# ginkgo-project/ginkgo

Measured on AMD Instinct MI355X. Metric: CSR SpMV GB/s (27-pt 3D Laplacian 256^3, fp64/int32), higher is better.
Workload: dtype f64

## Files before the change

ginkgo_amd/csrc/csr_offsets.hpp:

```cpp
#pragma once
#include "common.hpp"
#include <type_traits>

namespace gkoc {

constexpr int OFFS_MAX = 32;
constexpr int OFFS_TAB = OFFS_MAX + 1;

#ifdef __HIPCC__

template <typename I>
__global__ __launch_bounds__(256) void csr_offsets_build_kernel(int64_t n_rows, const I* __restrict__ row_ptrs,
                                                                const I* __restrict__ cols,
                                                                int32_t* __restrict__ seg_tab,
                                                                uint32_t* __restrict__ row_mask)
{
    const int64_t seg = int64_t(blockIdx.x) * 4 + threadIdx.x / 64;
    const int lane = threadIdx.x % 64;
    if (seg * 64 >= n_rows) return;
    const int64_t row = seg * 64 + lane;
    const bool valid = row < n_rows;
    int64_t pos = valid ? int64_t(row_ptrs[row]) : 0;
    const int64_t end = valid ? int64_t(row_ptrs[row + 1]) : 0;
    constexpr long long NONE = 0x7fffffffffffffffll;
    uint32_t mask = 0;
    int D = 0;
    int32_t my_off = 0;
    bool ok = true;
    long long last = 0;
    for (;;) {
        const long long cur = pos < end ? (long long)(cols[pos]) - (long long)(row) : NONE;
        long long m = cur;
#pragma unroll
        for (int o = 32; o > 0; o >>= 1) {
            const long long t = __shfl_xor(m, o, 64);
            m = t < m ? t : m;
        }
        if (m == NONE) break;
        if (D == OFFS_MAX || (D > 0 && m <= last) || m < -2147483648ll || m > 2147483647ll) {
            ok = false;
            break;
        }
        if (lane == D) my_off = int32_t(m);
        if (cur == m) {
            mask |= 1u << D;
            ++pos;
        }
        last = m;
        ++D;
    }
    if (!ok) D = 0;
    if (lane == 0) seg_tab[seg * OFFS_TAB] = D;
    if (lane < OFFS_MAX) seg_tab[seg * OFFS_TAB + 1 + lane] = lane < D ? my_off : 0;
    if (valid) row_mask[row] = ok ? mask : 0u;
}

__global__ __launch_bounds__(1024) void csr_offsets_finish_kernel(int64_t n_seg, const int32_t* __restrict__ seg_tab,
                                                                  const uint32_t* __restrict__ long_bits,
                                                                  uint32_t* __restrict__ skip,
                                                                  unsigned long long* __restrict__ count)
{
    __shared__ long long part[16];
    const int64_t n_words = (n_seg + 31) / 32;
    long long mine = 0;
    for (int64_t w = threadIdx.x; w < n_words; w += 1024) {
        uint32_t bits = 0;
        for (int j = 0; j < 32; ++j) {
            const int64_t s = w * 32 + j;
            if (s < n_seg && seg_tab[s * OFFS_TAB] > 0) bits |= 1u << j;
        }
        mine += __popc(bits);
        skip[w] = long_bits != nullptr ? (bits | long_bits[w]) : bits;
    }
    const long long total = block_sum<1024>(mine, part);
    if (threadIdx.x == 0) *count = static_cast<unsigned long long>(total);
}

template <typename T, bool ADV, bool DOT>
__global__ __launch_bounds__(64, 2) void csr_spmv_pipe3_kernel_offsets(
    int32_t n_rows, int32_t n_cols, int64_t n_segments, int spw, const int32_t* __restrict__ row_ptrs,
    const T* __restrict__ vals, const T* __restrict__ x, T* __restrict__ c, const T* __restrict__ alpha_p,
    const T* __restrict__ beta_p, const int32_t* __restrict__ seg_tab, const uint32_t* __restrict__ row_mask,
    T* __restrict__ dot_partial)
{
    constexpr int GR = 64;
    constexpr int E = 16 / sizeof(T);
    constexpr int CAP = GR * OFFS_MAX;
    constexpr int NL = CAP / (64 * E) + 1;
    constexpr int GPS = 64 / GR;
    typedef T VT __attribute__((ext_vector_type(E)));
    __shared__ __attribute__((aligned(16))) T stage[CAP + E];

    const int lane = threadIdx.x;
    const int64_t wave_id = blockIdx.x;
    const int64_t sb = wave_id * spw;
    const int n_units = int((sb + spw < n_segments ? int64_t(spw) : n_segments - sb)) * GPS;
    T alpha = T(1), beta = T(0);
    if (ADV) {
        alpha = alpha_p[0];
        beta = beta_p[0];
    }
    T dot_acc = T(0);

    struct unit {
        int D;
        int row0;
        int k0a, len;
        const int32_t* tab;
    };
    auto unit_of = [&](int u) {
        unit q;
        const int64_t s = sb + u / GPS;
        q.row0 = int(s * 64) + (u % GPS) * GR;
        q.tab = seg_tab + s * OFFS_TAB;
        q.D = (u < n_units && q.row0 < n_rows) ? q.tab[0] : 0;
        q.k0a = q.len = 0;
        if (q.D > 0) {
            const int last = q.row0 + GR < n_rows ? q.row0 + GR : n_rows;
            const int k0 = row_ptrs[q.row0];
            const int k1 = row_ptrs[last];
            q.k0a = k0 & ~(E - 1);
            q.len = k1 > k0 ? k1 - q.k0a : 0;
            if (q.len > CAP + E - 1) q.len = CAP + E - 1;
        }
        return q;
    };
    VT v[NL];
    auto load_vals = [&](const unit& q) {
        const int last_chunk = (q.len - 1) & ~(E - 1);
#pragma unroll
        for (int t = 0; t < NL; ++t) {
            const int k = (t * 64 + lane) * E;
            v[t] = *reinterpret_cast<const VT*>(vals + (int64_t(q.k0a) + (k < last_chunk ? k : last_chunk)));
        }
    };
    auto group = [&](auto nd_c, const unit& cur, const unit& nxt, int u) {
        constexpr int ND = decltype(nd_c)::value;
        const int row = cur.row0 + lane;
        const bool valid = lane < GR && row < n_rows;
        const int last = cur.row0 + GR < n_rows ? cur.row0 + GR : n_rows;
        const int rs = row_ptrs[valid ? row : last] - cur.k0a;
        uint32_t mask = row_mask[valid ? row : cur.row0];
        if (!valid) mask = 0u;
        T sum = T(0), bdot = T(0);
        if (ADV && beta != T(0)) sum = c[valid ? row : cur.row0] * beta;
        if (DOT) bdot = x[valid ? row : cur.row0];
        const int ncm1 = n_cols - 1;
        T xv[ND];
#pragma unroll
        for (int d = 0; d < ND; ++d) {
            const int idx = int(uint32_t(row) + uint32_t(cur.tab[1 + d]));
            xv[d] = x[idx < 0 ? 0 : (idx > ncm1 ? ncm1 : idx)];
        }
        if (cur.len > 0) {
#pragma unroll
            for (int t = 0; t < NL; ++t) {
                const int k = (t * 64 + lane) * E;
                if (k < cur.len) *reinterpret_cast<VT*>(&stage[k]) = v[t];
            }
        }
        wave_lds_sync();
        if (nxt.D > 0 && nxt.len > 0) load_vals(nxt);
#pragma unroll
        for (int d0 = 0; d0 < ND; d0 += 8) {
            T val[8];
#pragma unroll
            for (int i = 0; i < 8; ++i) {
                const int pos = rs + __popc(mask & ((1u << (d0 + i)) - 1u));
                val[i] = stage[pos];
            }
#pragma unroll
            for (int i = 0; i < 8; ++i) {
                asm volatile("" : "+v"(val[i]));
            }
#pragma unroll
            for (int i = 0; i < 8; ++i) {
                const T pr = ADV ? (alpha * val[i]) * xv[d0 + i] : val[i] * xv[d0 + i];
                sum = ((mask >> (d0 + i)) & 1u) != 0 ? sum + pr : sum;
            }
        }
        if (valid) c[row] = sum;
        if constexpr (DOT) {
            const T term = bdot * sum;
            if (valid) dot_acc += term;
        }
        wave_lds_sync();
    };

    unit cur = unit_of(0);
    if (cur.D > 0 && cur.len > 0) load_vals(cur);
    for (int u = 0; u < n_units; ++u) {
        const unit nxt = unit_of(u + 1);
        if (cur.D > 8) {
            group(std::integral_constant<int, OFFS_MAX>{}, cur, nxt, u);
        } else if (cur.D > 0) {
            group(std::integral_constant<int, 8>{}, cur, nxt, u);
        } else if (nxt.D > 0 && nxt.len > 0) {
            load_vals(nxt);
        }
        cur = nxt;
    }
    if constexpr (DOT) {
        dot_acc = wave_sum(dot_acc);
        if (lane == 0) dot_partial[wave_id] = dot_acc;
    }
}

#endif

}
```

ginkgo_amd/csrc/csr_spmv.hip:

```cpp
#include <algorithm>
#include <atomic>
#include <map>
#include <mutex>
#include <tuple>
#include <type_traits>
#include <vector>

#include "common.hpp"
#include "csr_long_rows.hpp"
#include "csr_offsets.hpp"
#include "csr_spmv_multi.hpp"
#include "csr_spmv_pipe.hpp"
#include "fused.hpp"

namespace gkoc {
namespace {

std::mutex g_long_mtx;
struct long_entry {
    csr_long_info info;
    std::vector<std::pair<hipStream_t, void*>> partials;
};
std::map<std::tuple<int, const void*, int64_t>, long_entry> g_long_cache;
std::atomic<int> g_long_cached{0};
constexpr size_t long_cache_cap = 128;
constexpr int64_t long_list_cap = 4096;

thread_local bool t_long_releasing = false;

void long_info_release(long_entry& en)
{
    csr_long_info& f = en.info;
    t_long_releasing = true;
    if (f.bits) (void)gkoc_free(f.bits);
    if (f.list) (void)gkoc_free(f.list);
    for (auto& sp : en.partials) (void)gkoc_free(sp.second);
    en.partials.clear();
    f = csr_long_info{};
    t_long_releasing = false;
}

bool stream_is_capturing(hipStream_t st)
{
    hipStreamCaptureStatus cap = hipStreamCaptureStatusNone;
    if (hipStreamIsCapturing(st, &cap) != hipSuccess || cap != hipStreamCaptureStatusNone) {
        (void)hipGetLastError();
        return true;
    }
    return false;
}

void long_partial_for(long_entry& en, hipStream_t st, csr_long_info* out)
{
    *out = en.info;
    if (en.info.count <= 0) return;
    for (auto& sp : en.partials) {
        if (sp.first == st) {
            out->partial = sp.second;
            return;
        }
    }
    void* p = nullptr;
    if (stream_is_capturing(st) ||
        gkoc_malloc(&p, size_t(en.info.count) * LONG_MAX_PER_SEG * LONG_PARTS * 8) != GKOC_OK) {
        (void)hipGetLastError();
        *out = csr_long_info{};
        out->nnz = en.info.nnz;
        return;
    }
    en.partials.emplace_back(st, p);
    out->partial = p;
}

template <typename T, typename I>
int long_info_of(gkoc_stream_t s, int64_t n_rows, const I* row_ptrs, csr_long_info* out)
{
    int dev = 0;
    GKOC_HIP(hipGetDevice(&dev));
    const auto key = std::make_tuple(dev, static_cast<const void*>(row_ptrs), n_rows);
    std::lock_guard<std::mutex> g(g_long_mtx);
    auto it = g_long_cache.find(key);
    if (it != g_long_cache.end()) {
        long_partial_for(it->second, as_stream(s), out);
        return GKOC_OK;
    }
    if (stream_is_capturing(as_stream(s))) {
        *out = csr_long_info{};
        return GKOC_OK;
    }
    if (g_long_cache.size() >= long_cache_cap) {
        auto oldest = g_long_cache.begin();
        for (auto jt = g_long_cache.begin(); jt != g_long_cache.end(); ++jt) {
            if (jt->second.info.seq < oldest->second.info.seq) oldest = jt;
        }
        if (oldest->second.info.count > 0) GKOC_HIP(hipDeviceSynchronize());
        long_info_release(oldest->second);
        g_long_cache.erase(oldest);
    }
    csr_long_info f;
    static uint64_t arrivals = 0;
    f.seq = ++arrivals;
    const int64_t n_seg = ceildiv(n_rows, int64_t(64));
    const size_t bit_bytes = size_t(ceildiv(n_seg, int64_t(32))) * 4;
    const size_t list_bytes = size_t(1 + long_list_cap) * 8;
    void *bits = nullptr, *list = nullptr;
    GKOC_TRY(gkoc_malloc(&bits, bit_bytes));
    if (gkoc_malloc(&list, list_bytes) != GKOC_OK) {
        t_long_releasing = true;
        (void)gkoc_free(bits);
        t_long_releasing = false;
        return GKOC_E_INVALID;
    }
    hipStream_t st = as_stream(s);
    unsigned long long count = 0;
    I nnz_dev = I(0);
    bool ok = hipMemsetAsync(bits, 0, bit_bytes, st) == hipSuccess && hipMemsetAsync(list, 0, 8, st) == hipSuccess;
    if (ok) {
        csr_long_row_scan_kernel<I><<<dim3(unsigned(ceildiv(n_seg, int64_t(4)))), dim3(256), 0, st>>>(
            n_rows, row_ptrs, static_cast<uint32_t*>(bits), static_cast<unsigned long long*>(list), long_list_cap);
        ok = hipGetLastError() == hipSuccess &&
             hipMemcpyAsync(&count, list, 8, hipMemcpyDeviceToHost, st) == hipSuccess &&
             hipMemcpyAsync(&nnz_dev, row_ptrs + n_rows, sizeof(I), hipMemcpyDeviceToHost, st) == hipSuccess &&
             hipStreamSynchronize(st) == hipSuccess;
    }
    if (ok) f.nnz = int64_t(nnz_dev);
    if (!ok || count == 0 || int64_t(count) > long_list_cap) {
        (void)hipGetLastError();
        t_long_releasing = true;
        (void)gkoc_free(bits);
        (void)gkoc_free(list);
        t_long_releasing = false;
    } else {
        f.count = int64_t(count);
        f.bits = static_cast<uint32_t*>(bits);
        f.list = static_cast<unsigned long long*>(list);
    }
    long_entry& en = g_long_cache[key];
    en.info = f;
    g_long_cached.store(int(g_long_cache.size()));
    long_partial_for(en, st, out);
    return GKOC_OK;
}

}

void csr_long_rows_forget(const void* ptr)
{
    if (ptr == nullptr || t_long_releasing || g_long_cached.load(std::memory_order_relaxed) == 0) return;
    std::vector<long_entry> gone;
    {
        std::lock_guard<std::mutex> g(g_long_mtx);
        for (auto it = g_long_cache.begin(); it != g_long_cache.end();) {
            if (std::get<1>(it->first) == ptr) {
                gone.push_back(it->second);
                it = g_long_cache.erase(it);
            } else {
                ++it;
            }
        }
        g_long_cached.store(int(g_long_cache.size()));
    }
    for (auto& en : gone) {
        if (en.info.count > 0) (void)hipDeviceSynchronize();
        long_info_release(en);
    }
}

std::atomic<int> g_csr_offsets_cached{0};

namespace {

template <int N>
using int_c = std::integral_constant<int, N>;

struct segment_plan {
    int64_t n_seg;
    int spw;
    int64_t n_waves;
};

int plan_segments(int64_t n_rows, segment_plan* plan, int64_t forced_spw = 0)
{
    const int64_t n_seg = ceildiv(n_rows, 64);
    const int spw = (forced_spw == 1 || forced_spw == 2) ? int(forced_spw) : (n_seg < 65536 ? 1 : 2);
    const int64_t n_waves = ceildiv(n_seg, spw);
    GKOC_REQUIRE(n_waves < (int64_t(1) << 31), GKOC_E_NOT_SUPPORTED, "more than 2^31 row segments");
    *plan = segment_plan{n_seg, spw, n_waves};
    return GKOC_OK;
}

template <typename F>
void with_store_mode(int spw, F&& launch)
{
    if (spw == 2) {
        launch(int_c<0x2000>{});
    } else {
        launch(int_c<0x1000>{});
    }
}

template <typename V, typename I>
bool streams_aligned(const V* vals, const I* cols, int E)
{
    return reinterpret_cast<uintptr_t>(vals) % (E * sizeof(V)) == 0 &&
           reinterpret_cast<uintptr_t>(cols) % (E * sizeof(I)) == 0;
}

template <typename T>
struct pipe_layout {
    static constexpr int EV = 32 / sizeof(T);
    static constexpr int RINGV = 8192 / sizeof(T);
    static constexpr int PE = sizeof(T) == 8 ? 2 : 4, PU = sizeof(T) == 8 ? 3 : 2;
};

template <typename T, typename I, bool ADV>
int launch_csr_columns(gkoc_stream_t s, int64_t n_rows, int64_t n_cols, const T* alpha, const I* row_ptrs,
                       const I* col_idxs, const T* vals, const T* b, int64_t ldb, const T* beta, T* c,
                       int64_t ldc, int64_t nrhs)
{
    const bool idx32 = n_cols * ldb < (int64_t(1) << 32);
    const bool pairs_ok = reinterpret_cast<uintptr_t>(b) % (2 * sizeof(T)) == 0 && ldb % 2 == 0 &&
                          reinterpret_cast<uintptr_t>(c) % (2 * sizeof(T)) == 0 && ldc % 2 == 0;
    const int64_t chunk_rows = tune_value(GKOC_TUNE_MULTI_XCD_CHUNK_ROWS);
    auto launch = [&](auto nr, auto cpl, auto ku, auto pipelined) -> int {
        constexpr int NR = decltype(nr)::value, CPL = decltype(cpl)::value, KU = decltype(ku)::value;
        constexpr bool PIPE = decltype(pipelined)::value;
        constexpr int rows = 64 * CPL / NR, segs = PIPE ? 4 : 1;
        const int64_t nwg = ceildiv(ceildiv(n_rows, rows), segs);
        GKOC_REQUIRE(nwg < (int64_t(1) << 31), GKOC_E_NOT_SUPPORTED, "more than 2^31 waves");
        const dim3 grid(static_cast<unsigned>(nwg)), block(64);
        auto go = [&](auto idx) {
            constexpr bool IDX32 = decltype(idx)::value;
            if constexpr (PIPE) {
                csr_spmv_frag_pipe_kernel<T, I, ADV, NR, CPL, KU, IDX32><<<grid, block, 0, as_stream(s)>>>(
                    n_rows, row_ptrs, col_idxs, vals, b, ldb, c, ldc, static_cast<int>(nrhs), alpha, beta, segs,
                    chunk_rows / (rows * segs));
            } else {
                csr_spmv_frag_kernel<T, I, ADV, NR, CPL, KU, IDX32><<<grid, block, 0, as_stream(s)>>>(
                    n_rows, row_ptrs, col_idxs, vals, b, ldb, c, ldc, static_cast<int>(nrhs), alpha, beta,
                    chunk_rows / rows);
            }
        };
        if (idx32) {
            go(std::true_type{});
        } else {
            go(std::false_type{});
        }
        GKOC_LAUNCH_OK();
        return GKOC_OK;
    };
    if (nrhs <= 4) return launch(int_c<4>{}, int_c<1>{}, int_c<4>{}, std::true_type{});
    if (pairs_ok) return launch(int_c<8>{}, int_c<2>{}, int_c<3>{}, std::true_type{});
    return launch(int_c<8>{}, int_c<1>{}, int_c<4>{}, std::false_type{});
}

template <typename T, typename I, bool ADV>
int launch_csr_pair(gkoc_stream_t s, int64_t n_rows, const T* alpha, const I* row_ptrs, const I* col_idxs,
                    const T* vals, const T* b, int64_t ldb, const T* beta, T* c, int64_t ldc)
{
    using lay = pipe_layout<T>;
    segment_plan p;
    GKOC_TRY(plan_segments(n_rows, &p));
    const dim3 grid(static_cast<unsigned>(p.n_waves)), block(64);
    const int b_vec_ok = reinterpret_cast<uintptr_t>(b) % (2 * sizeof(T)) == 0 && ldb % 2 == 0;
    const int64_t xcd_chunk = tune_value(GKOC_TUNE_MULTI_XCD_CHUNK_ROWS) / (64 * p.spw);
    auto launch = [&](auto e, auto u) {
        csr_spmv_multi_kernel<T, I, ADV, decltype(e)::value, decltype(u)::value, lay::RINGV / 2, 2>
            <<<grid, block, 0, as_stream(s)>>>(n_rows, p.n_seg, p.spw, row_ptrs, col_idxs, vals, b, ldb, c, ldc, 2,
                                               alpha, beta, b_vec_ok, xcd_chunk);
    };
    if (tune_value(GKOC_TUNE_CSR_LOAD_GROUPS) == 1) {
        launch(int_c<lay::EV>{}, int_c<1>{});
    } else {
        launch(int_c<lay::EV / 2>{}, int_c<2>{});
    }
    GKOC_LAUNCH_OK();
    return GKOC_OK;
}

std::mutex g_off_mtx;
struct offsets_plan {
    int state = 0;
    int64_t n_seg = 0, eligible = 0;
    int32_t* seg_tab = nullptr;
    uint32_t* row_mask = nullptr;
    uint32_t* skip = nullptr;
    bool with_long = false;
    int64_t bytes = 0, products = 0;
    uint64_t seq = 0;
    size_t rp_bytes = 0, ci_bytes = 0;
};
using offsets_key = std::tuple<int, const void*, const void*, int64_t>;
std::map<offsets_key, offsets_plan> g_off_cache;
constexpr size_t offsets_cache_cap = 128;
constexpr int64_t offsets_min_share = 50;

std::vector<void*> g_off_graveyard;

void offsets_release(std::vector<offsets_plan>& gone)
{
    std::vector<void*> bufs;
    for (auto& pl : gone) {
        for (void* b : {static_cast<void*>(pl.seg_tab), static_cast<void*>(pl.row_mask), static_cast<void*>(pl.skip)}) {
            if (b) bufs.push_back(b);
        }
    }
    if (bufs.empty()) return;
    std::lock_guard<std::mutex> g(g_off_mtx);
    g_off_graveyard.insert(g_off_graveyard.end(), bufs.begin(), bufs.end());
    if (hipDeviceSynchronize() != hipSuccess) {
        (void)hipGetLastError();
        return;
    }
    for (void* b : g_off_graveyard) (void)arena_free(b);
    g_off_graveyard.clear();
}

int offsets_build(hipStream_t st, int64_t n_rows, const int32_t* row_ptrs, const int32_t* col_idxs,
                  const csr_long_info& lng, offsets_plan& pl)
{
    const int64_t n_seg = ceildiv(n_rows, int64_t(64));
    const size_t tab_bytes = size_t(n_seg) * OFFS_TAB * 4, mask_bytes = size_t(n_rows) * 4;
    const size_t skip_bytes = size_t(ceildiv(n_seg, int64_t(32))) * 4;
    void *tab = nullptr, *mask = nullptr, *skip = nullptr, *count_dev = nullptr;
    bool ok = arena_malloc(&tab, tab_bytes, GKOC_MEM_INDICES) == GKOC_OK &&
              arena_malloc(&mask, mask_bytes, GKOC_MEM_INDICES) == GKOC_OK &&
              arena_malloc(&skip, skip_bytes, GKOC_MEM_INDICES) == GKOC_OK &&
              arena_malloc(&count_dev, 8, GKOC_MEM_VECTOR) == GKOC_OK;
    unsigned long long count = 0;
    if (ok) {
        csr_offsets_build_kernel<int32_t><<<dim3(unsigned(ceildiv(n_seg, int64_t(4)))), dim3(256), 0, st>>>(
            n_rows, row_ptrs, col_idxs, static_cast<int32_t*>(tab), static_cast<uint32_t*>(mask));
        csr_offsets_finish_kernel<<<dim3(1), dim3(1024), 0, st>>>(
            n_seg, static_cast<const int32_t*>(tab), lng.count > 0 ? lng.bits : nullptr,
            static_cast<uint32_t*>(skip), static_cast<unsigned long long*>(count_dev));
        ok = hipGetLastError() == hipSuccess &&
             hipMemcpyAsync(&count, count_dev, 8, hipMemcpyDeviceToHost, st) == hipSuccess &&
             hipStreamSynchronize(st) == hipSuccess;
    }
    (void)hipGetLastError();
    if (count_dev) (void)arena_free(count_dev);
    pl.n_seg = n_seg;
    pl.eligible = ok ? int64_t(count) : 0;
    if (!ok || pl.eligible == 0 || pl.eligible * 100 < n_seg * offsets_min_share) {
        if (tab) (void)arena_free(tab);
        if (mask) (void)arena_free(mask);
        if (skip) (void)arena_free(skip);
        if (ok) pl.state = 2;
        return GKOC_OK;
    }
    pl.state = 1;
    pl.seg_tab = static_cast<int32_t*>(tab);
    pl.row_mask = static_cast<uint32_t*>(mask);
    pl.bytes = int64_t(tab_bytes + mask_bytes);
    if (pl.eligible == n_seg) {
        (void)arena_free(skip);
    } else {
        pl.skip = static_cast<uint32_t*>(skip);
        pl.with_long = lng.count > 0;
        pl.bytes += int64_t(skip_bytes);
    }
    return GKOC_OK;
}

struct evicted_plans {
    std::vector<offsets_plan> v;
    ~evicted_plans() { offsets_release(v); }
};

offsets_plan* offsets_plan_for(hipStream_t st, int64_t n_rows, int64_t n_cols, const int32_t* row_ptrs,
                               const int32_t* col_idxs, const csr_long_info& lng, std::vector<offsets_plan>* evicted)
{
    const int64_t mode = tune_value(GKOC_TUNE_CSR_OFFSETS);
    if (mode == 2 || row_ptrs == nullptr || col_idxs == nullptr || n_cols < 1 ||
        n_rows >= (int64_t(1) << 31) - 64 || n_cols >= (int64_t(1) << 31)) {
        return nullptr;
    }
    int dev = 0;
    if (hipGetDevice(&dev) != hipSuccess) return nullptr;
    const offsets_key key{dev, row_ptrs, col_idxs, n_rows};
    auto it = g_off_cache.find(key);
    if (it == g_off_cache.end()) {
        const size_t rp_bytes = arena_allocation_bytes(row_ptrs), ci_bytes = arena_allocation_bytes(col_idxs);
        if (rp_bytes == 0 || ci_bytes == 0) return nullptr;
        if (g_off_cache.size() >= offsets_cache_cap) {
            auto oldest = g_off_cache.begin();
            for (auto jt = g_off_cache.begin(); jt != g_off_cache.end(); ++jt) {
                if (jt->second.seq < oldest->second.seq) oldest = jt;
            }
            evicted->push_back(oldest->second);
            g_off_cache.erase(oldest);
        }
        static uint64_t arrivals = 0;
        offsets_plan fresh;
        fresh.seq = ++arrivals;
        fresh.rp_bytes = rp_bytes;
        fresh.ci_bytes = ci_bytes;
        it = g_off_cache.emplace(key, fresh).first;
        g_csr_offsets_cached.store(int(g_off_cache.size()));
        if (mode != 1) return nullptr;
    }
    offsets_plan& pl = it->second;
    if (pl.state == 0) {
        if (stream_is_capturing(st)) return nullptr;
        (void)offsets_build(st, n_rows, row_ptrs, col_idxs, lng, pl);
    }
    if (pl.state != 1) return nullptr;
    if (pl.skip != nullptr && pl.with_long != (lng.count > 0)) return nullptr;
    return &pl;
}

template <typename T, bool ADV, bool DOT>
void launch_offsets_kernel(hipStream_t st, const offsets_plan& pl, const segment_plan& p, int64_t n_rows,
                           int64_t n_cols, const T* alpha, const int32_t* row_ptrs, const T* vals, const T* b,
                           const T* beta, T* c, T* dot_partial)
{
    const dim3 grid(static_cast<unsigned>(p.n_waves)), block(64);
    csr_spmv_pipe3_kernel_offsets<T, ADV, DOT><<<grid, block, 0, st>>>(
        int32_t(n_rows), int32_t(n_cols), p.n_seg, p.spw, row_ptrs, vals, b, c, alpha, beta, pl.seg_tab,
        pl.row_mask, dot_partial);
}

template <typename T, typename I, bool ADV>
int launch_hub_rows(hipStream_t st, const csr_long_info& lng, int64_t n_rows, const T* alpha, const I* row_ptrs,
                    const I* col_idxs, const T* vals, const T* b, int64_t ldb, const T* beta, T* c, int64_t ldc)
{
    csr_flagged_segments_kernel<T, I, ADV><<<dim3(unsigned(lng.count * LONG_PARTS)), dim3(LONG_WG), 0, st>>>(
        n_rows, row_ptrs, col_idxs, vals, b, ldb, c, ldc, alpha, beta, lng.list, static_cast<T*>(lng.partial));
    GKOC_LAUNCH_OK();
    csr_long_rows_fold_kernel<T, I, ADV><<<dim3(unsigned(lng.count)), dim3(64), 0, st>>>(
        n_rows, row_ptrs, c, ldc, beta, lng.list, static_cast<const T*>(lng.partial));
    GKOC_LAUNCH_OK();
    return GKOC_OK;
}

template <typename T, typename I, bool ADV>
int launch_csr_single(gkoc_stream_t s, int64_t n_rows, int64_t n_cols, const T* alpha, const I* row_ptrs, const I* col_idxs,
                      const T* vals, const T* b, int64_t ldb, const T* beta, T* c, int64_t ldc, int64_t nrhs)
{
    using lay = pipe_layout<T>;
    csr_long_info lng;
    if (nrhs == 1 && tune_value(GKOC_TUNE_CSR_LONG_ROWS) != 0) {
        GKOC_TRY((long_info_of<T, I>(s, n_rows, row_ptrs, &lng)));
    }
    const uint32_t* seg_skip = lng.count > 0 ? lng.bits : nullptr;
    constexpr bool offsets_type = std::is_same<I, int32_t>::value && (sizeof(T) == 8 || sizeof(T) == 4);
    evicted_plans evicted;
    std::unique_lock<std::mutex> plan_lock(g_off_mtx, std::defer_lock);
    offsets_plan* plan = nullptr;
    if constexpr (offsets_type) {
        if (nrhs == 1 && ldb == 1 && ldc == 1 && vals != nullptr && b != nullptr &&
            reinterpret_cast<uintptr_t>(vals) % 16 == 0 && tune_value(GKOC_TUNE_CSR_OFFSETS) != 2) {
            plan_lock.lock();
            plan = offsets_plan_for(as_stream(s), n_rows, n_cols, row_ptrs, col_idxs, lng, &evicted.v);
            if (plan == nullptr) plan_lock.unlock();
        }
    }
    segment_plan p;
    GKOC_TRY(plan_segments(n_rows, &p, tune_value(GKOC_TUNE_CSR_SEGS_PER_WAVE)));
    const dim3 grid(static_cast<unsigned>(p.n_waves)), block(64);
    if constexpr (offsets_type) {
        if (plan != nullptr) {
            launch_offsets_kernel<T, ADV, false>(as_stream(s), *plan, p, n_rows, n_cols, alpha, row_ptrs, vals, b,
                                                 beta, c, static_cast<T*>(nullptr));
            GKOC_LAUNCH_OK();
            ++plan->products;
            if (plan->skip == nullptr) return GKOC_OK;
            seg_skip = plan->skip;
        }
    }
    const int64_t xcd_choice = tune_value(GKOC_TUNE_CSR_XCD_MAP);
    const int xcd_map =
        ((xcd_choice == 1 || (xcd_choice == 0 && lng.count > 0)) && p.n_waves >= 8 * 1024) ? 1 : 0;
    const bool vec_ok = streams_aligned(vals, col_idxs, lay::EV);
    const int64_t groups = tune_value(GKOC_TUNE_CSR_LOAD_GROUPS);
    const bool long_float_rows = sizeof(T) == 4 && lng.nnz > 0 && lng.nnz >= 40 * n_rows;
    with_store_mode(p.spw, [&](auto mode) {
        auto launch = [&](auto e, auto u) {
            csr_spmv_pipe3_kernel<T, I, ADV, 64, decltype(e)::value, decltype(u)::value, lay::RINGV, 1,
                                  decltype(mode)::value><<<grid, block, 0, as_stream(s)>>>(
                n_rows, p.n_seg, p.spw, row_ptrs, col_idxs, vals, b, ldb, c, ldc, static_cast<int>(nrhs), alpha,
                beta, nullptr, xcd_map, static_cast<const I*>(nullptr), static_cast<int*>(nullptr), int64_t(0),
                int64_t(0), static_cast<const uint32_t*>(nullptr), uint32_t(0), static_cast<const I*>(nullptr),
                static_cast<const I*>(nullptr), static_cast<const T*>(nullptr), static_cast<uint32_t*>(nullptr),
                uint32_t(0), 0, int64_t(-1), seg_skip);
        };
        if (!vec_ok) {
            launch(int_c<1>{}, int_c<4>{});
        } else if (groups == 3 || (groups == 0 && long_float_rows)) {
            launch(int_c<1>{}, int_c<8>{});
        } else if (groups == 4) {
            launch(int_c<2>{}, int_c<4>{});
        } else if (groups == 1 || p.n_seg < 32768) {
            launch(int_c<lay::EV>{}, int_c<1>{});
        } else {
            launch(int_c<lay::PE>{}, int_c<lay::PU>{});
        }
    });
    GKOC_LAUNCH_OK();
    if (lng.count > 0) {
        GKOC_TRY((launch_hub_rows<T, I, ADV>(as_stream(s), lng, n_rows, alpha, row_ptrs, col_idxs, vals, b, ldb,
                                             beta, c, ldc)));
    }
    return GKOC_OK;
}

template <typename T, typename I, bool ADV>
int launch_csr(gkoc_stream_t s, int64_t n_rows, int64_t n_cols, const T* alpha,
               const I* row_ptrs, const I* col_idxs, const T* vals, const T* b,
               int64_t ldb, const T* beta, T* c, int64_t ldc, int64_t nrhs)
{
    GKOC_REQUIRE(n_rows >= 0 && n_cols >= 0 && nrhs >= 0, GKOC_E_INVALID,
                 "negative dimension");
    if (n_rows == 0 || nrhs == 0) return GKOC_OK;
    GKOC_REQUIRE(row_ptrs && c, GKOC_E_INVALID, "null pointer");
    GKOC_REQUIRE(ldc >= nrhs && (n_cols == 0 || ldb >= nrhs), GKOC_E_INVALID,
                 "stride smaller than nrhs");
    if (ADV) GKOC_REQUIRE(alpha && beta, GKOC_E_INVALID, "null alpha/beta");
    if (nrhs >= 3) {
        return launch_csr_columns<T, I, ADV>(s, n_rows, n_cols, alpha, row_ptrs, col_idxs, vals, b, ldb, beta, c,
                                             ldc, nrhs);
    }
    if (nrhs == 2 && streams_aligned(vals, col_idxs, pipe_layout<T>::EV)) {
        return launch_csr_pair<T, I, ADV>(s, n_rows, alpha, row_ptrs, col_idxs, vals, b, ldb, beta, c, ldc);
    }
    return launch_csr_single<T, I, ADV>(s, n_rows, n_cols, alpha, row_ptrs, col_idxs, vals, b, ldb, beta, c, ldc, nrhs);
}

__global__ void gate_open_kernel(uint32_t* gate, uint32_t epoch)
{
    __hip_atomic_store(gate, epoch, __ATOMIC_RELEASE, __HIP_MEMORY_SCOPE_SYSTEM);
}

int64_t gated_wave_cap() { return int64_t(current_device_props().num_cu) * 8; }

bool gated_fits(int64_t n_rows, int64_t head_rows, int64_t tail_rows)
{
    if (n_rows <= 0 || head_rows < 0 || tail_rows < 0 || head_rows + tail_rows > n_rows ||
        head_rows + tail_rows == 0) {
        return false;
    }
    return ceildiv(head_rows + tail_rows, 64) <= gated_wave_cap();
}

template <typename T, typename I>
int launch_csr_gated(gkoc_stream_t s, int64_t n_rows, const I* row_ptrs, const I* col_idxs, const T* vals,
                     const I* bnd_ptrs, const I* bnd_cols, const T* bnd_vals, const T* b, T* c,
                     int64_t head_rows, int64_t tail_rows, const uint32_t* gate, uint32_t epoch,
                     uint32_t* fork_word, uint32_t fork_number, T* dot_out = nullptr, void* work = nullptr,
                     size_t work_bytes = 0)
{
    GKOC_REQUIRE(n_rows > 0 && head_rows >= 0 && tail_rows >= 0 && head_rows + tail_rows <= n_rows,
                 GKOC_E_INVALID, "bad dimensions");
    GKOC_REQUIRE(head_rows + tail_rows > 0, GKOC_E_INVALID, "no boundary rows: use gkoc_csr_spmv_*");
    GKOC_REQUIRE(row_ptrs && col_idxs && vals && bnd_ptrs && bnd_cols && bnd_vals && b && c && gate,
                 GKOC_E_INVALID, "null pointer");
    GKOC_REQUIRE(gated_fits(n_rows, head_rows, tail_rows), GKOC_E_NOT_SUPPORTED,
                 "more boundary rows than may wait on the device at once (gkoc_csr_spmv_gated_fits): "
                 "use the join-based product");
    using lay = pipe_layout<T>;
    GKOC_REQUIRE(streams_aligned(vals, col_idxs, lay::EV) && streams_aligned(bnd_vals, bnd_cols, lay::EV),
                 GKOC_E_NOT_SUPPORTED, "values / column indices not aligned for vector loads");
    const int64_t n_int = ceildiv(n_rows - head_rows - tail_rows, 64);
    const int64_t n_bnd = ceildiv(head_rows + tail_rows, 64);
    GKOC_REQUIRE(n_int + n_bnd < (int64_t(1) << 31), GKOC_E_NOT_SUPPORTED, "more than 2^31 row segments");
    T* partial = nullptr;
    if (dot_out) {
        GKOC_REQUIRE(work && work_bytes >= fused_workspace_bytes(n_rows + 128, sizeof(T)), GKOC_E_WORKSPACE,
                     "workspace too small (gkoc_x_workspace_bytes(n_rows + 128))");
        partial = static_cast<T*>(work);
    }
    const dim3 grid(static_cast<unsigned>(n_int + n_bnd)), block(64);
    const int gate_fence = std::max(
        gate_fence_policy(),
        (tune_value(GKOC_TUNE_GATE_FENCE) != 0 || reinterpret_cast<uintptr_t>(b) % 128 != 0) ? 1 : 0);
    int64_t pos = tune_value(GKOC_TUNE_GATE_POS);
    if (pos < 0 || pos > 100) pos = 100;
    const int64_t bnd_first = pos >= 100 ? -1 : n_int * pos / 100;
    const bool wide = tune_value(GKOC_TUNE_CSR_LOAD_GROUPS) == 1;
    auto launch = [&](auto mode) {
        auto go = [&](auto e, auto u) {
            csr_spmv_pipe3_kernel<T, I, false, 64, decltype(e)::value, decltype(u)::value, lay::RINGV, 1,
                                  decltype(mode)::value><<<grid, block, 0, as_stream(s)>>>(
                n_rows, n_int + n_bnd, 1, row_ptrs, col_idxs, vals, b, 1, c, 1, 1, nullptr, nullptr, partial, 0,
                nullptr, nullptr, head_rows, tail_rows, gate, epoch, bnd_ptrs, bnd_cols, bnd_vals, fork_word,
                fork_number, gate_fence, bnd_first);
        };
        if (wide) {
            go(int_c<lay::EV>{}, int_c<1>{});
        } else {
            go(int_c<lay::PE>{}, int_c<lay::PU>{});
        }
    };
    if (dot_out) {
        launch(int_c<0x11040>{});
    } else {
        launch(int_c<0x11000>{});
    }
    GKOC_LAUNCH_OK();
    if (dot_out) {
        fold_partials_wide_kernel<T><<<dim3(1), dim3(fold_block), 0, as_stream(s)>>>(n_int + n_bnd, partial,
                                                                                      dot_out);
        GKOC_LAUNCH_OK();
    }
    return GKOC_OK;
}

__global__ void delay_kernel(long long ticks)
{
    extern __shared__ char delay_lds[];
    if (threadIdx.x == 0) delay_lds[0] = 0;
    const long long t0 = wall_clock64();
    while (wall_clock64() - t0 < ticks) __builtin_amdgcn_s_sleep(64);
}

template <typename T, typename V, typename I, bool ADV>
int launch_csr_mixed(gkoc_stream_t s, int64_t n_rows, int64_t n_cols, const T* alpha,
                     const I* row_ptrs, const I* col_idxs, const V* vals, const T* b, int64_t ldb,
                     const T* beta, T* c, int64_t ldc, int64_t nrhs)
{
    GKOC_REQUIRE(n_rows >= 0 && n_cols >= 0 && nrhs >= 0, GKOC_E_INVALID, "negative dimension");
    if (n_rows == 0 || nrhs == 0) return GKOC_OK;
    GKOC_REQUIRE(row_ptrs && c, GKOC_E_INVALID, "null pointer");
    GKOC_REQUIRE(ldc >= nrhs && (n_cols == 0 || ldb >= nrhs), GKOC_E_INVALID,
                 "stride smaller than nrhs");
    if (ADV) GKOC_REQUIRE(alpha && beta, GKOC_E_INVALID, "null alpha/beta");
    using lay = pipe_layout<T>;
    segment_plan p;
    GKOC_TRY(plan_segments(n_rows, &p));
    const dim3 grid(static_cast<unsigned>(p.n_waves)), block(64);
    const bool vec_ok = streams_aligned(vals, col_idxs, lay::EV);
    with_store_mode(p.spw, [&](auto mode) {
        auto launch = [&](auto e, auto u) {
            csr_spmv_pipe3_kernel<T, I, ADV, 64, decltype(e)::value, decltype(u)::value, lay::RINGV, 1,
                                  decltype(mode)::value, V><<<grid, block, 0, as_stream(s)>>>(
                n_rows, p.n_seg, p.spw, row_ptrs, col_idxs, vals, b, ldb, c, ldc, static_cast<int>(nrhs), alpha,
                beta, nullptr, 0);
        };
        if (vec_ok) {
            launch(int_c<lay::EV>{}, int_c<1>{});
        } else {
            launch(int_c<1>{}, int_c<4>{});
        }
    });
    GKOC_LAUNCH_OK();
    return GKOC_OK;
}

template <typename T, typename I>
int launch_csr_dot(gkoc_stream_t s, int64_t n, const I* row_ptrs,
                   const I* col_idxs, const T* vals, const T* b, T* c,
                   T* dot_out, void* work, size_t work_bytes)
{
    GKOC_REQUIRE(n >= 0, GKOC_E_INVALID, "negative dimension");
    GKOC_REQUIRE(dot_out, GKOC_E_INVALID, "null result");
    if (n == 0) {
        GKOC_HIP(hipMemsetAsync(dot_out, 0, sizeof(T), as_stream(s)));
        return GKOC_OK;
    }
    GKOC_REQUIRE(row_ptrs && b && c && work, GKOC_E_INVALID, "null pointer");
    GKOC_REQUIRE(work_bytes >= fused_workspace_bytes(n, sizeof(T)), GKOC_E_WORKSPACE,
                 "workspace too small (gkoc_x_workspace_bytes)");
    if (tune_value(GKOC_TUNE_CSR_LONG_ROWS) != 0) {
        csr_long_info lng;
        GKOC_TRY((long_info_of<T, I>(s, n, row_ptrs, &lng)));
        if (lng.count > 0) {
            GKOC_TRY((launch_csr<T, I, false>(s, n, n, nullptr, row_ptrs, col_idxs, vals, b, 1, nullptr, c, 1, 1)));
            if constexpr (sizeof(T) == 8) {
                return gkoc_dense_compute_dot_f64(s, n, 1, reinterpret_cast<const double*>(b), 1,
                                                  reinterpret_cast<const double*>(c), 1,
                                                  reinterpret_cast<double*>(dot_out), work, work_bytes);
            } else {
                return gkoc_dense_compute_dot_f32(s, n, 1, reinterpret_cast<const float*>(b), 1,
                                                  reinterpret_cast<const float*>(c), 1,
                                                  reinterpret_cast<float*>(dot_out), work, work_bytes);
            }
        }
    }
    using lay = pipe_layout<T>;
    segment_plan p;
    GKOC_TRY(plan_segments(n, &p));
    T* partial = static_cast<T*>(work);
    T* scratch = partial + (fused_workspace_bytes(n, sizeof(T)) / sizeof(T) - fold_chunks);
    const dim3 grid(static_cast<unsigned>(p.n_waves)), block(64);
    const bool vec_ok = streams_aligned(vals, col_idxs, 4);
    const int xcd_map = (tune_value(GKOC_TUNE_CSR_XCD_MAP) == 1 && p.n_waves >= 8 * 1024) ? 1 : 0;
    if constexpr (std::is_same<I, int32_t>::value) {
        if (vals != nullptr && reinterpret_cast<uintptr_t>(vals) % 16 == 0 && tune_value(GKOC_TUNE_CSR_OFFSETS) != 2) {
            evicted_plans evicted;
            std::lock_guard<std::mutex> plan_lock(g_off_mtx);
            offsets_plan* plan = offsets_plan_for(as_stream(s), n, n, row_ptrs, col_idxs, csr_long_info{}, &evicted.v);
            if (plan != nullptr && plan->skip == nullptr) {
                launch_offsets_kernel<T, false, true>(as_stream(s), *plan, p, n, n, static_cast<const T*>(nullptr),
                                                      row_ptrs, vals, b, static_cast<const T*>(nullptr), c, partial);
                GKOC_LAUNCH_OK();
                ++plan->products;
                return fold_partials<T>(s, p.n_waves, partial, scratch, dot_out, false);
            }
        }
    }
    constexpr int DOT_WPS = sizeof(I) == 4 ? 4 : 1;
    with_store_mode(p.spw, [&](auto mode) {
        auto launch = [&](auto e, auto u) {
            csr_spmv_pipe3_kernel<T, I, false, 64, decltype(e)::value, decltype(u)::value, 1024, DOT_WPS,
                                  (decltype(mode)::value | 0x40)><<<grid, block, 0, as_stream(s)>>>(
                n, p.n_seg, p.spw, row_ptrs, col_idxs, vals, b, 1, c, 1, 1, nullptr, nullptr, partial, xcd_map);
        };
        if (vec_ok) {
            launch(int_c<lay::PE>{}, int_c<lay::PU>{});
        } else {
            launch(int_c<1>{}, int_c<4>{});
        }
    });
    GKOC_LAUNCH_OK();
    return fold_partials<T>(s, p.n_waves, partial, scratch, dot_out, false);
}


constexpr int row_stage_cap = 2048;

template <typename I>
struct row_segment {
    int64_t row, rs, re, K0, K1;
    bool valid;
};

template <typename I>
__device__ __forceinline__ row_segment<I> load_row_segment(int64_t n_rows,
                                                           const I* row_ptrs)
{
    row_segment<I> g;
    const int64_t first = int64_t(blockIdx.x) * 64;
    g.row = first + threadIdx.x;
    g.valid = g.row < n_rows;
    const int64_t last = first + 64 < n_rows ? first + 64 : n_rows;
    g.rs = row_ptrs[g.valid ? g.row : last];
    g.re = row_ptrs[g.valid ? g.row + 1 : last];
    g.K0 = row_ptrs[first];
    g.K1 = row_ptrs[last];
    return g;
}

template <typename T, typename I>
__global__ __launch_bounds__(64) void extract_diag_kernel(
    int64_t n_diag, const I* __restrict__ row_ptrs, const I* __restrict__ cols,
    const T* __restrict__ vals, T* __restrict__ diag)
{
    __shared__ I lc[row_stage_cap];
    const row_segment<I> g = load_row_segment<I>(n_diag, row_ptrs);
    const bool staged = g.K1 - g.K0 <= row_stage_cap;
    if (staged) {
        for (int i = threadIdx.x; i < int(g.K1 - g.K0); i += 64) lc[i] = cols[g.K0 + i];
        wave_lds_sync();
    }
    if (!g.valid) return;
    T d = T(0);
    for (int64_t k = g.rs; k < g.re; ++k) {
        const I c = staged ? lc[k - g.K0] : cols[k];
        if (int64_t(c) == g.row) {
            d = vals[k];
            break;
        }
    }
    diag[g.row] = d;
}

template <typename I>
__global__ __launch_bounds__(64) void is_sorted_kernel(
    int64_t n_rows, const I* __restrict__ row_ptrs, const I* __restrict__ cols,
    int* __restrict__ flag)
{
    __shared__ I lc[row_stage_cap];
    const row_segment<I> g = load_row_segment<I>(n_rows, row_ptrs);
    const bool staged = g.K1 - g.K0 <= row_stage_cap;
    if (staged) {
        for (int i = threadIdx.x; i < int(g.K1 - g.K0); i += 64) lc[i] = cols[g.K0 + i];
        wave_lds_sync();
    }
    bool ok = true;
    if (g.valid) {
        for (int64_t k = g.rs + 1; k < g.re; ++k) {
            const I a = staged ? lc[k - 1 - g.K0] : cols[k - 1];
            const I b = staged ? lc[k - g.K0] : cols[k];
            if (a > b) {
                ok = false;
                break;
            }
        }
    }
    if (__any(!ok) && threadIdx.x == 0) atomicAnd(flag, 0);
}

template <typename T, typename I>
__global__ __launch_bounds__(64) void sort_rows_kernel(
    int64_t n_rows, const I* __restrict__ row_ptrs, I* __restrict__ cols,
    T* __restrict__ vals)
{
    __shared__ I lc[row_stage_cap];
    __shared__ T lv[row_stage_cap];
    const row_segment<I> g = load_row_segment<I>(n_rows, row_ptrs);
    const bool staged = g.K1 - g.K0 <= row_stage_cap;
    if (staged) {
        const int seg = int(g.K1 - g.K0);
        for (int i = threadIdx.x; i < seg; i += 64) {
            lc[i] = cols[g.K0 + i];
            lv[i] = vals[g.K0 + i];
        }
        wave_lds_sync();
        if (g.valid) {
            const int a = int(g.rs - g.K0), e = int(g.re - g.K0);
            for (int i = a + 1; i < e; ++i) {
                const I ci = lc[i];
                const T vi = lv[i];
                int k = i - 1;
                while (k >= a && lc[k] > ci) {
                    lc[k + 1] = lc[k];
                    lv[k + 1] = lv[k];
                    --k;
                }
                lc[k + 1] = ci;
                lv[k + 1] = vi;
            }
        }
        wave_lds_sync();
        for (int i = threadIdx.x; i < seg; i += 64) {
            cols[g.K0 + i] = lc[i];
            vals[g.K0 + i] = lv[i];
        }
        return;
    }
    if (!g.valid) return;
    for (int64_t i = g.rs + 1; i < g.re; ++i) {
        const I ci = cols[i];
        const T vi = vals[i];
        int64_t k = i - 1;
        while (k >= g.rs && cols[k] > ci) {
            cols[k + 1] = cols[k];
            vals[k + 1] = vals[k];
            --k;
        }
        cols[k + 1] = ci;
        vals[k + 1] = vi;
    }
}

}

void csr_offsets_forget(const void* first, size_t bytes)
{
    const char* lo = static_cast<const char*>(first);
    const char* hi = lo + (bytes ? bytes : 1);
    std::vector<offsets_plan> gone;
    {
        std::lock_guard<std::mutex> g(g_off_mtx);
        for (auto it = g_off_cache.begin(); it != g_off_cache.end();) {
            const char* rp = static_cast<const char*>(std::get<1>(it->first));
            const char* ci = static_cast<const char*>(std::get<2>(it->first));
            if ((lo < rp + it->second.rp_bytes && rp < hi) || (lo < ci + it->second.ci_bytes && ci < hi)) {
                gone.push_back(it->second);
                it = g_off_cache.erase(it);
            } else {
                ++it;
            }
        }
        g_csr_offsets_cached.store(int(g_off_cache.size()));
    }
    offsets_release(gone);
}

template <typename T, typename I>
int csr_spmv_complex(gkoc_stream_t s, int64_t n_rows, int64_t nrhs, const I* row_ptrs, const I* col_idxs,
                     const T* vals, const T* alpha, const T* b, int64_t ldb, const T* beta, T* c, int64_t ldc)
{
    if (n_rows <= 0 || nrhs <= 0) return GKOC_OK;
    GKOC_REQUIRE(row_ptrs && c, GKOC_E_INVALID, "null pointer");
    GKOC_REQUIRE(nrhs <= 0x7fffffff, GKOC_E_NOT_SUPPORTED, "more than 2^31 right-hand sides");
    if (col_idxs == nullptr || vals == nullptr || b == nullptr) return GKOC_E_NOT_SUPPORTED;
    constexpr int E = sizeof(T) == 16 ? 1 : 2, U = sizeof(T) == 16 ? 4 : 2;
    if (!streams_aligned(vals, col_idxs, E) || reinterpret_cast<uintptr_t>(b) % sizeof(T) != 0 ||
        reinterpret_cast<uintptr_t>(c) % sizeof(T) != 0) {
        return GKOC_E_NOT_SUPPORTED;
    }
    segment_plan p;
    GKOC_TRY(plan_segments(n_rows, &p));
    const dim3 grid(static_cast<unsigned>(p.n_waves)), block(64);
    constexpr int CX_WPS = sizeof(I) == 4 ? 4 : 1;
    if (alpha != nullptr) GKOC_REQUIRE(beta != nullptr, GKOC_E_INVALID, "alpha and beta go together");
    with_store_mode(p.spw, [&](auto mode) {
        auto launch = [&](auto advanced) {
            constexpr bool ADV = decltype(advanced)::value;
            csr_spmv_pipe3_kernel<T, I, ADV, 64, E, U, pipe_layout<T>::RINGV, (ADV ? 1 : CX_WPS),
                                  decltype(mode)::value><<<grid, block, 0, as_stream(s)>>>(
                n_rows, p.n_seg, p.spw, row_ptrs, col_idxs, vals, b, ldb, c, ldc, static_cast<int>(nrhs), alpha,
                beta);
        };
        if (alpha != nullptr) {
            launch(std::true_type{});
        } else {
            launch(std::false_type{});
        }
    });
    GKOC_LAUNCH_OK();
    return GKOC_OK;
}
#define GKOC_INST_CX(T, I)                                                                                       \
    template int csr_spmv_complex<T, I>(gkoc_stream_t, int64_t, int64_t, const I*, const I*, const T*, const T*, \
                                        const T*, int64_t, const T*, T*, int64_t);
GKOC_INST_CX(gkoc_c128, int32_t)
GKOC_INST_CX(gkoc_c128, int64_t)
GKOC_INST_CX(gkoc_c64, int32_t)
GKOC_INST_CX(gkoc_c64, int64_t)
#undef GKOC_INST_CX

}

using namespace gkoc;

#define GKOC_DEF_CSR(T, TN, I, IN)                                             \
    extern "C" int gkoc_csr_spmv_##TN##_##IN(                                  \
        gkoc_stream_t s, int64_t n_rows, int64_t n_cols, const I* row_ptrs,    \
        const I* col_idxs, const T* vals, const T* b, int64_t ldb, T* c,       \
        int64_t ldc, int64_t nrhs)                                             \
    {                                                                          \
        return launch_csr<T, I, false>(s, n_rows, n_cols, nullptr, row_ptrs,   \
                                       col_idxs, vals, b, ldb, nullptr, c,     \
                                       ldc, nrhs);                             \
    }                                                                          \
    extern "C" int gkoc_csr_advanced_spmv_##TN##_##IN(                         \
        gkoc_stream_t s, int64_t n_rows, int64_t n_cols, const T* alpha,       \
        const I* row_ptrs, const I* col_idxs, const T* vals, const T* b,       \
        int64_t ldb, const T* beta, T* c, int64_t ldc, int64_t nrhs)           \
    {                                                                          \
        return launch_csr<T, I, true>(s, n_rows, n_cols, alpha, row_ptrs,      \
                                      col_idxs, vals, b, ldb, beta, c, ldc,    \
                                      nrhs);                                   \
    }                                                                          \
    extern "C" int gkoc_x_csr_spmv_dot_##TN##_##IN(                            \
        gkoc_stream_t s, int64_t n, const I* row_ptrs, const I* col_idxs,      \
        const T* vals, const T* b, T* c, T* dot_out, void* work,               \
        size_t work_bytes)                                                     \
    {                                                                          \
        return launch_csr_dot<T, I>(s, n, row_ptrs, col_idxs, vals, b, c,      \
                                    dot_out, work, work_bytes);                \
    }                                                                          \
    extern "C" int gkoc_csr_extract_diagonal_##TN##_##IN(                      \
        gkoc_stream_t s, int64_t n_rows, int64_t n_cols, const I* row_ptrs,    \
        const I* col_idxs, const T* vals, T* diag)                             \
    {                                                                          \
        const int64_t nd = n_rows < n_cols ? n_rows : n_cols;                  \
        if (nd <= 0) return GKOC_OK;                                           \
        extract_diag_kernel<T, I>                                              \
            <<<dim3(unsigned(ceildiv(nd, 64))), dim3(64), 0, as_stream(s)>>>(  \
                nd, row_ptrs, col_idxs, vals, diag);                           \
        GKOC_LAUNCH_OK();                                                      \
        return GKOC_OK;                                                        \
    }                                                                          \
    extern "C" int gkoc_csr_is_sorted_by_column_index_##TN##_##IN(             \
        gkoc_stream_t s, int64_t n_rows, const I* row_ptrs,                    \
        const I* col_idxs, int* is_sorted_host)                                \
    {                                                                          \
        GKOC_REQUIRE(is_sorted_host, GKOC_E_INVALID, "null result");           \
        *is_sorted_host = 1;                                                   \
        if (n_rows <= 0) return GKOC_OK;                                       \
        int* flag = nullptr;                                                   \
        GKOC_TRY(scratch_malloc(as_stream(s), reinterpret_cast<void**>(&flag), \
                                sizeof(int)));                                 \
         \
         \
        GKOC_HIP(hipMemsetAsync(flag, 1, sizeof(int), as_stream(s)));          \
        is_sorted_kernel<I>                                                    \
            <<<dim3(unsigned(ceildiv(n_rows, 64))), dim3(64), 0,               \
               as_stream(s)>>>(n_rows, row_ptrs, col_idxs, flag);              \
        GKOC_LAUNCH_OK();                                                      \
        GKOC_HIP(hipMemcpyAsync(is_sorted_host, flag, sizeof(int),             \
                                hipMemcpyDeviceToHost, as_stream(s)));         \
        GKOC_HIP(hipStreamSynchronize(as_stream(s)));                          \
        GKOC_TRY(scratch_free(as_stream(s), flag));                            \
        *is_sorted_host = *is_sorted_host != 0;                                \
        return GKOC_OK;                                                        \
    }                                                                          \
    extern "C" int gkoc_csr_sort_by_column_index_##TN##_##IN(                  \
        gkoc_stream_t s, int64_t n_rows, const I* row_ptrs, I* col_idxs,       \
        T* vals)                                                               \
    {                                                                          \
// ... 150 lines not shown
```

Measured before the change: 7932.

## Software-pipeline offsets SpMV kernel across segments and template on max diagonal count

Restructures the offsets-based CSR SpMV kernel into head/rows phases so the next segment's table, row pointers and values are fetched while the current segment's products are computed, with the per-segment offsets held in registers instead of reread from the table. The finish kernel now also records the maximum diagonal count, and the host uses it to pick an ND=8 or ND=32 template, removing runtime branching between group widths. Segments with no work are skipped in the pipeline loop. The cost is higher register pressure from carrying offsets and lane state, plus an extra atomic and a 16-byte readback during plan build. The dot path also now passes a segments-per-wave tune value.

```diff
diff --git a/ginkgo_amd/csrc/csr_offsets.hpp b/ginkgo_amd/csrc/csr_offsets.hpp
--- a/ginkgo_amd/csrc/csr_offsets.hpp
+++ b/ginkgo_amd/csrc/csr_offsets.hpp
@@ -61,22 +61,33 @@
                                                                   unsigned long long* __restrict__ count)
 {
     __shared__ long long part[16];
+    __shared__ int d_max;
+    if (threadIdx.x == 0) d_max = 0;
+    __syncthreads();
     const int64_t n_words = (n_seg + 31) / 32;
     long long mine = 0;
+    int my_d = 0;
     for (int64_t w = threadIdx.x; w < n_words; w += 1024) {
         uint32_t bits = 0;
         for (int j = 0; j < 32; ++j) {
             const int64_t s = w * 32 + j;
-            if (s < n_seg && seg_tab[s * OFFS_TAB] > 0) bits |= 1u << j;
+            const int D = s < n_seg ? seg_tab[s * OFFS_TAB] : 0;
+            if (D > 0) bits |= 1u << j;
+            my_d = D > my_d ? D : my_d;
         }
         mine += __popc(bits);
         skip[w] = long_bits != nullptr ? (bits | long_bits[w]) : bits;
     }
+    atomicMax(&d_max, my_d);
     const long long total = block_sum<1024>(mine, part);
-    if (threadIdx.x == 0) *count = static_cast<unsigned long long>(total);
-}
-
-template <typename T, bool ADV, bool DOT>
+    __syncthreads();
+    if (threadIdx.x == 0) {
+        count[0] = static_cast<unsigned long long>(total);
+        count[1] = static_cast<unsigned long long>(d_max);
+    }
+}
+
+template <typename T, bool ADV, bool DOT, int ND>
 __global__ __launch_bounds__(64, 2) void csr_spmv_pipe3_kernel_offsets(
     int32_t n_rows, int32_t n_cols, int64_t n_segments, int spw, const int32_t* __restrict__ row_ptrs,
     const T* __restrict__ vals, const T* __restrict__ x, T* __restrict__ c, const T* __restrict__ alpha_p,
@@ -87,14 +98,13 @@
     constexpr int E = 16 / sizeof(T);
     constexpr int CAP = GR * OFFS_MAX;
     constexpr int NL = CAP / (64 * E) + 1;
-    constexpr int GPS = 64 / GR;
     typedef T VT __attribute__((ext_vector_type(E)));
-    __shared__ __attribute__((aligned(16))) T stage[CAP + E];
+    __shared__ __attribute__((aligned(16))) T stage[NL * 64 * E];
 
     const int lane = threadIdx.x;
     const int64_t wave_id = blockIdx.x;
     const int64_t sb = wave_id * spw;
-    const int n_units = int((sb + spw < n_segments ? int64_t(spw) : n_segments - sb)) * GPS;
+    const int n_units = int(sb + spw < n_segments ? int64_t(spw) : n_segments - sb);
     T alpha = T(1), beta = T(0);
     if (ADV) {
         alpha = alpha_p[0];
@@ -103,28 +113,44 @@
     T dot_acc = T(0);
 
     struct unit {
+        int u;
         int D;
         int row0;
         int k0a, len;
-        const int32_t* tab;
-    };
-    auto unit_of = [&](int u) {
+        int32_t off[ND];
+    };
+    struct unit_raw {
+        int u, row0, k0, k1, D;
+        int32_t off[ND];
+    };
+    auto read_unit = [&](int u) {
+        unit_raw r;
+        r.u = u;
+        const int64_t s = sb + (u < n_units ? u : n_units - 1);
+        const int32_t* tab = seg_tab + s * OFFS_TAB;
+        r.row0 = int(s * 64);
+        const int last = r.row0 + GR < n_rows ? r.row0 + GR : n_rows;
+        r.k0 = row_ptrs[r.row0];
+        r.k1 = row_ptrs[last];
+        r.D = tab[0];
+#pragma unroll
+        for (int d = 0; d < ND; ++d) r.off[d] = tab[1 + d];
+        return r;
+    };
+    auto unit_from = [&](const unit_raw& r) {
         unit q;
-        const int64_t s = sb + u / GPS;
-        q.row0 = int(s * 64) + (u % GPS) * GR;
-        q.tab = seg_tab + s * OFFS_TAB;
-        q.D = (u < n_units && q.row0 < n_rows) ? q.tab[0] : 0;
-        q.k0a = q.len = 0;
-        if (q.D > 0) {
-            const int last = q.row0 + GR < n_rows ? q.row0 + GR : n_rows;
-            const int k0 = row_ptrs[q.row0];
-            const int k1 = row_ptrs[last];
-            q.k0a = k0 & ~(E - 1);
-            q.len = k1 > k0 ? k1 - q.k0a : 0;
-            if (q.len > CAP + E - 1) q.len = CAP + E - 1;
-        }
+        q.u = r.u;
+        q.D = r.D;
+        q.row0 = r.row0;
+#pragma unroll
+        for (int d = 0; d < ND; ++d) q.off[d] = r.off[d];
+        q.k0a = r.k0 & ~(E - 1);
+        int len = r.k1 - q.k0a;
+        if (len > CAP + E - 1) len = CAP + E - 1;
+        q.len = (r.u < n_units && r.D > 0 && r.D <= ND && r.k1 > r.k0) ? len : 0;
         return q;
     };
+    auto unit_of = [&](int u) { return unit_from(read_unit(u)); };
     VT v[NL];
     auto load_vals = [&](const unit& q) {
         const int last_chunk = (q.len - 1) & ~(E - 1);
@@ -134,35 +160,47 @@
             v[t] = *reinterpret_cast<const VT*>(vals + (int64_t(q.k0a) + (k < last_chunk ? k : last_chunk)));
         }
     };
-    auto group = [&](auto nd_c, const unit& cur, const unit& nxt, int u) {
-        constexpr int ND = decltype(nd_c)::value;
-        const int row = cur.row0 + lane;
-        const bool valid = lane < GR && row < n_rows;
+    struct lane_state {
+        int row, rs_raw;
+        bool valid;
+        uint32_t mask_raw;
+        T sum, bdot;
+        T xv[ND];
+    };
+    auto head = [&](const unit& cur, lane_state& ls, unit_raw& nxt_raw) {
+        ls.row = cur.row0 + lane;
+        ls.valid = ls.row < n_rows;
         const int last = cur.row0 + GR < n_rows ? cur.row0 + GR : n_rows;
-        const int rs = row_ptrs[valid ? row : last] - cur.k0a;
-        uint32_t mask = row_mask[valid ? row : cur.row0];
-        if (!valid) mask = 0u;
-        T sum = T(0), bdot = T(0);
-        if (ADV && beta != T(0)) sum = c[valid ? row : cur.row0] * beta;
-        if (DOT) bdot = x[valid ? row : cur.row0];
+        ls.rs_raw = row_ptrs[ls.valid ? ls.row : last];
+        ls.mask_raw = row_mask[ls.valid ? ls.row : cur.row0];
+        ls.sum = T(0);
+        ls.bdot = T(0);
+        if (ADV && beta != T(0)) ls.sum = c[ls.valid ? ls.row : cur.row0] * beta;
+        if (DOT) ls.bdot = x[ls.valid ? ls.row : cur.row0];
         const int ncm1 = n_cols - 1;
-        T xv[ND];
 #pragma unroll
         for (int d = 0; d < ND; ++d) {
-            const int idx = int(uint32_t(row) + uint32_t(cur.tab[1 + d]));
-            xv[d] = x[idx < 0 ? 0 : (idx > ncm1 ? ncm1 : idx)];
-        }
-        if (cur.len > 0) {
-#pragma unroll
-            for (int t = 0; t < NL; ++t) {
-                const int k = (t * 64 + lane) * E;
-                if (k < cur.len) *reinterpret_cast<VT*>(&stage[k]) = v[t];
-            }
-        }
+            const int idx = int(uint32_t(ls.row) + uint32_t(cur.off[d]));
+            ls.xv[d] = x[idx < 0 ? 0 : (idx > ncm1 ? ncm1 : idx)];
+        }
+        nxt_raw = read_unit(cur.u + 1);
+#pragma unroll
+        for (int t = 0; t < NL; ++t) *reinterpret_cast<VT*>(&stage[(t * 64 + lane) * E]) = v[t];
         wave_lds_sync();
-        if (nxt.D > 0 && nxt.len > 0) load_vals(nxt);
-#pragma unroll
-        for (int d0 = 0; d0 < ND; d0 += 8) {
+        __builtin_amdgcn_sched_barrier(0);
+    };
+    auto next_group = [&](const unit_raw& nxt_raw) {
+        unit nxt = unit_from(nxt_raw);
+        while (nxt.u < n_units && nxt.len == 0) nxt = unit_of(nxt.u + 1);
+        return nxt;
+    };
+    auto rows = [&](const unit& cur, lane_state& ls) {
+        __builtin_amdgcn_sched_barrier(0);
+        const int rs = ls.rs_raw - cur.k0a;
+        const uint32_t mask = ls.valid ? ls.mask_raw : 0u;
+        T sum = ls.sum;
+        auto slots = [&](auto d0_c) {
+            constexpr int d0 = decltype(d0_c)::value;
             T val[8];
 #pragma unroll
             for (int i = 0; i < 8; ++i) {
@@ -175,30 +213,43 @@
             }
 #pragma unroll
             for (int i = 0; i < 8; ++i) {
-                const T pr = ADV ? (alpha * val[i]) * xv[d0 + i] : val[i] * xv[d0 + i];
+                const T pr = ADV ? (alpha * val[i]) * ls.xv[d0 + i] : val[i] * ls.xv[d0 + i];
                 sum = ((mask >> (d0 + i)) & 1u) != 0 ? sum + pr : sum;
             }
-        }
-        if (valid) c[row] = sum;
+        };
+        slots(std::integral_constant<int, 0>{});
+        if constexpr (ND > 8) {
+            slots(std::integral_constant<int, 8>{});
+            slots(std::integral_constant<int, 16>{});
+            slots(std::integral_constant<int, 24>{});
+        }
+        asm volatile("" : "+v"(sum));
+        if (ls.valid) c[ls.row] = sum;
         if constexpr (DOT) {
-            const T term = bdot * sum;
-            if (valid) dot_acc += term;
+            const T term = ls.bdot * sum;
+            if (ls.valid) dot_acc += term;
         }
         wave_lds_sync();
     };
 
-    unit cur = unit_of(0);
-    if (cur.D > 0 && cur.len > 0) load_vals(cur);
-    for (int u = 0; u < n_units; ++u) {
-        const unit nxt = unit_of(u + 1);
-        if (cur.D > 8) {
-            group(std::integral_constant<int, OFFS_MAX>{}, cur, nxt, u);
-        } else if (cur.D > 0) {
-            group(std::integral_constant<int, 8>{}, cur, nxt, u);
-        } else if (nxt.D > 0 && nxt.len > 0) {
-            load_vals(nxt);
-        }
-        cur = nxt;
+    if (n_units > 0) {
+        unit cur = unit_of(0);
+        while (cur.u < n_units && cur.len == 0) cur = unit_of(cur.u + 1);
+        if (cur.u < n_units) {
+            lane_state ls;
+            unit_raw nxt_raw;
+            load_vals(cur);
+            head(cur, ls, nxt_raw);
+            unit nxt = next_group(nxt_raw);
+            while (nxt.u < n_units) {
+                load_vals(nxt);
+                rows(cur, ls);
+                cur = nxt;
+                head(cur, ls, nxt_raw);
+                nxt = next_group(nxt_raw);
+            }
+            rows(cur, ls);
+        }
     }
     if constexpr (DOT) {
         dot_acc = wave_sum(dot_acc);
diff --git a/ginkgo_amd/csrc/csr_spmv.hip b/ginkgo_amd/csrc/csr_spmv.hip
--- a/ginkgo_amd/csrc/csr_spmv.hip
+++ b/ginkgo_amd/csrc/csr_spmv.hip
@@ -282,6 +282,7 @@
 struct offsets_plan {
     int state = 0;
     int64_t n_seg = 0, eligible = 0;
+    int max_d = 0;
     int32_t* seg_tab = nullptr;
     uint32_t* row_mask = nullptr;
     uint32_t* skip = nullptr;
@@ -326,8 +327,8 @@
     bool ok = arena_malloc(&tab, tab_bytes, GKOC_MEM_INDICES) == GKOC_OK &&
               arena_malloc(&mask, mask_bytes, GKOC_MEM_INDICES) == GKOC_OK &&
               arena_malloc(&skip, skip_bytes, GKOC_MEM_INDICES) == GKOC_OK &&
-              arena_malloc(&count_dev, 8, GKOC_MEM_VECTOR) == GKOC_OK;
-    unsigned long long count = 0;
+              arena_malloc(&count_dev, 16, GKOC_MEM_VECTOR) == GKOC_OK;
+    unsigned long long count[2] = {0, 0};
     if (ok) {
         csr_offsets_build_kernel<int32_t><<<dim3(unsigned(ceildiv(n_seg, int64_t(4)))), dim3(256), 0, st>>>(
             n_rows, row_ptrs, col_idxs, static_cast<int32_t*>(tab), static_cast<uint32_t*>(mask));
@@ -335,13 +336,14 @@
             n_seg, static_cast<const int32_t*>(tab), lng.count > 0 ? lng.bits : nullptr,
             static_cast<uint32_t*>(skip), static_cast<unsigned long long*>(count_dev));
         ok = hipGetLastError() == hipSuccess &&
-             hipMemcpyAsync(&count, count_dev, 8, hipMemcpyDeviceToHost, st) == hipSuccess &&
+             hipMemcpyAsync(count, count_dev, 16, hipMemcpyDeviceToHost, st) == hipSuccess &&
              hipStreamSynchronize(st) == hipSuccess;
     }
     (void)hipGetLastError();
     if (count_dev) (void)arena_free(count_dev);
     pl.n_seg = n_seg;
-    pl.eligible = ok ? int64_t(count) : 0;
+    pl.eligible = ok ? int64_t(count[0]) : 0;
+    pl.max_d = ok ? int(count[1]) : 0;
     if (!ok || pl.eligible == 0 || pl.eligible * 100 < n_seg * offsets_min_share) {
         if (tab) (void)arena_free(tab);
         if (mask) (void)arena_free(mask);
@@ -416,9 +418,15 @@
                            const T* beta, T* c, T* dot_partial)
 {
     const dim3 grid(static_cast<unsigned>(p.n_waves)), block(64);
-    csr_spmv_pipe3_kernel_offsets<T, ADV, DOT><<<grid, block, 0, st>>>(
-        int32_t(n_rows), int32_t(n_cols), p.n_seg, p.spw, row_ptrs, vals, b, c, alpha, beta, pl.seg_tab,
-        pl.row_mask, dot_partial);
+    if (pl.max_d > 8) {
+        csr_spmv_pipe3_kernel_offsets<T, ADV, DOT, OFFS_MAX><<<grid, block, 0, st>>>(
+            int32_t(n_rows), int32_t(n_cols), p.n_seg, p.spw, row_ptrs, vals, b, c, alpha, beta, pl.seg_tab,
+            pl.row_mask, dot_partial);
+    } else {
+        csr_spmv_pipe3_kernel_offsets<T, ADV, DOT, 8><<<grid, block, 0, st>>>(
+            int32_t(n_rows), int32_t(n_cols), p.n_seg, p.spw, row_ptrs, vals, b, c, alpha, beta, pl.seg_tab,
+            pl.row_mask, dot_partial);
+    }
 }
 
 template <typename T, typename I, bool ADV>
@@ -679,7 +687,7 @@
     }
     using lay = pipe_layout<T>;
     segment_plan p;
-    GKOC_TRY(plan_segments(n, &p));
+    GKOC_TRY(plan_segments(n, &p, tune_value(GKOC_TUNE_CSR_SEGS_PER_WAVE)));
     T* partial = static_cast<T*>(work);
     T* scratch = partial + (fused_workspace_bytes(n, sizeof(T)) / sizeof(T) - fold_chunks);
     const dim3 grid(static_cast<unsigned>(p.n_waves)), block(64);
```

Result: faster. 8318, median of 6 (+4.9%).
